# gardnerzhou/CHAP

Hardware: AMD Instinct MI355X
Metric: training volumes/sec (2D 256^2 bs24) (higher is better)
Workload: dtype bf16; 1 GPU; ACDC 2D DualDecoder bs=24 (12 lab + 12 unlab) 256x256, 1 perturb step(s), N_v=U; global_batch=24, parallelism=dp1, hip_graph=True, losses_finite=True

## Files before the change

### chap_amd/csrc/actbwd_math.h

```cpp
#pragma once
#include "common.h"

typedef float actbwd_f32x2 __attribute__((ext_vector_type(2)));

__device__ __forceinline__ void actbwd_consts8(const float a0[8], const float a1[8], const float gm[8], const float mean[8], const float istd[8], float count,
                                               float k0[8], float cB[8], float cC[8]) {
#pragma unroll
    for (int j = 0; j < 8; ++j) {
        k0[j] = gm[j] * istd[j];
        const float k1 = a0[j] / count, k2 = a1[j] / count;
        cB[j] = -istd[j] * k0[j] * k2;
        cC[j] = __builtin_fmaf(mean[j] * istd[j] * k0[j], k2, -k0[j] * k1);
    }
}

__device__ __forceinline__ void actbwd_deriv8(const float raw[8], const float dy[8], const float sa[8], const float sb[8], bool act, float slope, float dz[8]) {
    if (act) {
#pragma unroll
        for (int j = 0; j < 4; ++j) {
            const actbwd_f32x2 r2 = {raw[2 * j], raw[2 * j + 1]}, a2 = {sa[2 * j], sa[2 * j + 1]}, b2 = {sb[2 * j], sb[2 * j + 1]};
            const actbwd_f32x2 z = __builtin_elementwise_fma(r2, a2, b2);
            const actbwd_f32x2 f = {z.x > 0.f ? 1.f : slope, z.y > 0.f ? 1.f : slope};
            const actbwd_f32x2 g2 = {dy[2 * j], dy[2 * j + 1]};
            const actbwd_f32x2 d = g2 * f;
            dz[2 * j] = d.x; dz[2 * j + 1] = d.y;
        }
    } else {
#pragma unroll
        for (int j = 0; j < 8; ++j) dz[j] = dy[j];
    }
}
__device__ __forceinline__ void actbwd_keep8(float dz[8], uint2 m, float keep_scale) {
#pragma unroll
    for (int j = 0; j < 8; ++j) {
        const uint32_t w = j < 4 ? m.x : m.y;
        dz[j] = ((w >> (8 * (j & 3))) & 0xff) ? dz[j] * keep_scale : 0.f;
    }
}

__device__ __forceinline__ void actbwd_apply8(const float dz[8], const float raw[8], const float k0[8], const float cB[8], const float cC[8], float o[8]) {
#pragma unroll
    for (int j = 0; j < 4; ++j) {
        const actbwd_f32x2 d = {dz[2 * j], dz[2 * j + 1]}, r2 = {raw[2 * j], raw[2 * j + 1]};
        const actbwd_f32x2 A = {k0[2 * j], k0[2 * j + 1]}, B = {cB[2 * j], cB[2 * j + 1]}, Cc = {cC[2 * j], cC[2 * j + 1]};
        const actbwd_f32x2 r = __builtin_elementwise_fma(d, A, __builtin_elementwise_fma(r2, B, Cc));
        o[2 * j] = r.x; o[2 * j + 1] = r.y;
    }
}
```

### chap_amd/csrc/pointwise.hip

```cpp
#include <cstdlib>
#include "common.h"
#include "launch.h"
#include "actbwd_math.h"
#include "conv_c1_mfma.h"

typedef unsigned int u32;

__device__ __forceinline__ double wave_sum_f64(double v) {
#pragma unroll
    for (int o = 32; o > 0; o >>= 1) v += __shfl_xor(v, o, 64);
    return v;
}

template <typename T, bool D3, int CO>
__device__ __forceinline__ void conv_c1_fwd_kernel(const chap_conv_c1_params& P) {
    constexpr int KD = D3 ? 3 : 1, TAPS = KD * 9;
    __shared__ float ws[CO * TAPS + 2 * CO];
    __shared__ float bstat[4][2 * CO];
    for (int i = threadIdx.x; i < CO * TAPS; i += 256) ws[i] = P.w[i];
    for (int i = threadIdx.x; i < CO; i += 256) { ws[CO * TAPS + i] = P.bias ? P.bias[i] : 0.f; ws[CO * TAPS + CO + i] = (P.stats && P.stats_shift) ? P.stats_shift[i] : 0.f; }
    __syncthreads();
    const long npix = (long)P.N * P.D * P.H * P.W;
    float ssum[CO], ssq[CO];
#pragma unroll
    for (int c = 0; c < CO; ++c) { ssum[c] = 0.f; ssq[c] = 0.f; }
    for (long pix = (long)blockIdx.x * 256 + threadIdx.x; pix < npix; pix += (long)gridDim.x * 256) {
        const u32 up = (u32)pix;
        const int x = (int)(up % (u32)P.W); u32 r = up / (u32)P.W;
        const int y = (int)(r % (u32)P.H); r /= (u32)P.H;
        const int z = (int)(r % (u32)P.D); const int n = (int)(r / (u32)P.D);
        float in[TAPS];
#pragma unroll
        for (int dz = 0; dz < KD; ++dz)
#pragma unroll
            for (int dy = 0; dy < 3; ++dy)
#pragma unroll
                for (int dx = 0; dx < 3; ++dx) {
                    const int zz = z + dz - (D3 ? 1 : 0), yy = y + dy - 1, xx = x + dx - 1;
                    const bool ib = (unsigned)zz < (unsigned)P.D && (unsigned)yy < (unsigned)P.H && (unsigned)xx < (unsigned)P.W;
                    in[(dz * 3 + dy) * 3 + dx] = ib ? P.x[(((long)n * P.D + zz) * P.H + yy) * P.W + xx] : 0.f;
                }
        float acc[CO];
#pragma unroll
        for (int c = 0; c < CO; ++c) {
            float a = ws[CO * TAPS + c];
#pragma unroll
            for (int t = 0; t < TAPS; ++t) a = fmaf(in[t], ws[c * TAPS + t], a);
            acc[c] = a;
            const float as = a - ws[CO * TAPS + CO + c];
            ssum[c] += as; ssq[c] += as * as;
        }
        T* o = (T*)P.out + pix * CO;
#pragma unroll
        for (int c = 0; c < CO; c += 8) st8(o + c, acc + c);
    }
    if (P.stats) {
#pragma unroll
        for (int c = 0; c < CO; ++c) {
            const float s = wave_sum(ssum[c]), q = wave_sum(ssq[c]);
            if ((threadIdx.x & 63) == 0) { bstat[threadIdx.x >> 6][c] = s; bstat[threadIdx.x >> 6][CO + c] = q; }
        }
        __syncthreads();
        if (blockIdx.x == 0 && threadIdx.x == 0) *(int*)P.stats = (int)gridDim.x;
        for (int i = threadIdx.x; i < 2 * CO; i += 256)
// ... 112 lines not shown
            P.ws[(long)blockIdx.x * (CO * TAPS + CO) + i] = part[0][i] + part[1][i] + part[2][i] + part[3][i];
    }
}

struct c1_reduce_args { const float* ws; int nblocks, taps; float* dw; float* db; };
template <int CO>
__device__ __forceinline__ void conv_c1_reduce_kernel(const c1_reduce_args& A) {
    const float* ws = A.ws; const int nblocks = A.nblocks, taps = A.taps; float* dw = A.dw; float* db = A.db;
    __shared__ float red[4];
    const int i = blockIdx.x;
    const int tot = CO * taps + CO;
    float s = 0.f;
    for (int b = threadIdx.x; b < nblocks; b += 256) s += ws[(long)b * tot + i];
    s = wave_sum(s);
    if ((threadIdx.x & 63) == 0) red[threadIdx.x >> 6] = s;
    __syncthreads();
    if (threadIdx.x == 0) {
        s = (red[0] + red[1]) + (red[2] + red[3]);
        if (i < CO * taps) { if (dw) dw[i] += s; } else if (db) db[i - CO * taps] += s;
    }
}

static int c1_bwd_blocks(const chap_conv_c1_bwd_params* p) {
    const long npix = (long)p->N * p->D * p->H * p->W;
    long b = (npix + 255) / 256;
    return (int)(b < 1024 ? b : 1024);
}
extern "C" size_t chap_conv_c1_bwd_ws(const chap_conv_c1_bwd_params* p) {
    const int taps = p->dims == 3 ? 27 : 9;
    return (size_t)c1_bwd_blocks(p) * (p->Cout * taps + p->Cout) * sizeof(float);
}
extern "C" int chap_conv_c1_bwd(const chap_conv_c1_bwd_params* p, void* stream) {
    CHAP_CHECK_ARG(p && p->g && p->w, "chap_conv_c1_bwd: null argument");
    CHAP_CHECK_ARG(p->Cout == 16, "chap_conv_c1_bwd: Cout=%d (only 16 built)", p->Cout);
    CHAP_CHECK_ARG(!(p->dw || p->db) || (p->ws && p->x), "chap_conv_c1_bwd: dw/db need x and ws");
    const int nb = c1_bwd_blocks(p);
    hipStream_t s = (hipStream_t)stream;
    const bool d3 = p->dims == 3, bf = p->dtype == CHAP_BF16;
    const c1_bwd_args a = {*p, nb};
    int r;
    if (bf && d3) r = chap_launch<c1_bwd_args, conv_c1_bwd_kernel<bf16_t, true, 16>, 256>(dim3(nb), dim3(256), 0, s, a, "chap_conv_c1_bwd");
    else if (bf) r = chap_launch<c1_bwd_args, conv_c1_bwd_kernel<bf16_t, false, 16>, 256>(dim3(nb), dim3(256), 0, s, a, "chap_conv_c1_bwd");
    else if (d3) r = chap_launch<c1_bwd_args, conv_c1_bwd_kernel<float, true, 16>, 256>(dim3(nb), dim3(256), 0, s, a, "chap_conv_c1_bwd");
    else r = chap_launch<c1_bwd_args, conv_c1_bwd_kernel<float, false, 16>, 256>(dim3(nb), dim3(256), 0, s, a, "chap_conv_c1_bwd");
    if (r) return r;
    if (p->dw || p->db) {
        const int taps = d3 ? 27 : 9, tot = 16 * taps + 16;
        const c1_reduce_args ra = {(const float*)p->ws, nb, taps, p->dw, p->db};
        return chap_launch<c1_reduce_args, conv_c1_reduce_kernel<16>, 256>(dim3(tot), dim3(256), 0, s, ra, "chap_conv_c1_bwd(reduce)");
    }
    return CHAP_OK;
}

__device__ __forceinline__ void bn_finalize_kernel(const chap_bn_finalize_params& P) {
    const int c = blockIdx.x * 4 + (threadIdx.x >> 6), lane = threadIdx.x & 63;
    if (c >= P.C) return;
    const int nslots = *(const int*)P.stats;
    const bool upd = P.momentum > 0.f && P.running_mean;
    const float gam = P.gamma[c], bet = P.beta[c], sft = P.stats_shift ? P.stats_shift[c] : 0.f;
    const float rm0 = upd ? P.running_mean[c] : 0.f, rv0 = upd ? P.running_var[c] : 0.f;
    const int nsub = P.Clog / P.C;
    const float* st = P.stats + CHAP_STATS_HDR;
    double s = 0.0, q = 0.0;
    constexpr int NB = CHAP_STATS_MAX_SLOTS / 64;
    for (int k = 0; k < nsub; ++k) {
        float vs[NB], vq[NB];
#pragma unroll
        for (int i = 0; i < NB; ++i) {
            const int b = lane + 64 * i;
            const float* row = st + (long)(b < nslots ? b : 0) * 2 * P.Clog + k * P.C + c;
            vs[i] = row[0]; vq[i] = row[P.Clog];
        }
#pragma unroll
        for (int i = 0; i < NB; ++i) {
            const bool ok = lane + 64 * i < nslots;
            s += ok ? (double)vs[i] : 0.0; q += ok ? (double)vq[i] : 0.0;
        }
    }
    s = wave_sum_f64(s); q = wave_sum_f64(q);
    if (lane != 0) return;
    if (c == 0 && P.num_batches_tracked && P.momentum > 0.f) *P.num_batches_tracked += 1;
    const double cnt = (double)P.count;
    const double ms = s / cnt;
    double var = q / cnt - ms * ms;
    var = var > 0.0 ? var : 0.0;
    const float mean = (float)((double)sft + ms);
    const float invstd = (float)(1.0 / sqrt(var + (double)P.eps));
    const float sc = gam * invstd;
    P.scale[c] = sc;
    P.shift[c] = bet - mean * sc;
    if (P.mean) { P.mean[c] = mean; P.invstd[c] = invstd; }
    if (upd) {
        const float unb = (float)(cnt > 1.0 ? var * cnt / (cnt - 1.0) : var);
        P.running_mean[c] = (1.f - P.momentum) * rm0 + P.momentum * mean;
        P.running_var[c] = (1.f - P.momentum) * rv0 + P.momentum * unb;
    }
}
extern "C" int chap_bn_finalize(const chap_bn_finalize_params* p, void* stream) {
    CHAP_CHECK_ARG(p && p->stats && p->gamma && p->beta && p->scale && p->shift && p->C > 0 && p->count > 0, "chap_bn_finalize: bad argument");
    CHAP_CHECK_ARG(p->Clog >= p->C && p->Clog % p->C == 0, "chap_bn_finalize: Clog=%d must be a multiple of C=%d", p->Clog, p->C);
    if (chap_lab_skip(KNOB_LAB_SKIP_BNFIN)) return CHAP_OK;
    return chap_launch<chap_bn_finalize_params, bn_finalize_kernel, 256>(dim3(cdiv(p->C, 4)), dim3(256), 0, (hipStream_t)stream, *p, "chap_bn_finalize");
}

__device__ __forceinline__ void bn_eval_kernel(const chap_bn_eval_params& P) {
    const int c = blockIdx.x * blockDim.x + threadIdx.x;
    if (c >= P.C) return;
    const float sc = P.gamma[c] * rsqrtf(P.running_var[c] + P.eps);
    P.scale[c] = sc;
    P.shift[c] = P.beta[c] - P.running_mean[c] * sc;
}
extern "C" int chap_bn_eval_affine(const chap_bn_eval_params* p, void* stream) {
    CHAP_CHECK_ARG(p && p->gamma && p->beta && p->running_mean && p->running_var && p->scale && p->shift && p->C > 0, "chap_bn_eval_affine: bad argument");
    return chap_launch<chap_bn_eval_params, bn_eval_kernel, 64>(dim3(cdiv(p->C, 64)), dim3(64), 0, (hipStream_t)stream, *p, "chap_bn_eval_affine");
}

template <typename T>
__device__ __forceinline__ void act_pool2_kernel(const chap_pool_params& P) {
    const int D = P.D > 1 ? P.D : 1, KZ = P.D > 1 ? 2 : 1;
    const int C8 = P.r.C / 8, OD = D / KZ, OH = P.H / 2, OW = P.W / 2;
    const long total = (long)P.N * OD * OH * OW * C8;
    for (long i = (long)blockIdx.x * 256 + threadIdx.x; i < total; i += (long)gridDim.x * 256) {
        const u32 ui = (u32)i;
        const int c8 = (int)(ui % (u32)C8) * 8; u32 r = ui / (u32)C8;
        const int ox = (int)(r % (u32)OW); r /= (u32)OW;
        const int oy = (int)(r % (u32)OH); r /= (u32)OH;
        const int oz = (int)(r % (u32)OD); const int n = (int)(r / (u32)OD);
        float best[8]; uint32_t bi[8];
        for (int k = 0; k < 4 * KZ; ++k) {
            const long pix = (((long)n * D + KZ * oz + (k >> 2)) * P.H + 2 * oy + ((k >> 1) & 1)) * P.W + 2 * ox + (k & 1);
            float v[8];
            src_load8<T>(P.r, n, pix, c8, v);
#pragma unroll
            for (int j = 0; j < 8; ++j)
                if (k == 0 || v[j] > best[j] || v[j] != v[j]) { best[j] = v[j]; bi[j] = k; }
        }
        const long op = (((long)n * OD + oz) * OH + oy) * OW + ox;
        st8((T*)P.out + op * P.r.C + c8, best);
        if (P.idx) {
            uint2 m;
            m.x = bi[0] | (bi[1] << 8) | (bi[2] << 16) | (bi[3] << 24);
            m.y = bi[4] | (bi[5] << 8) | (bi[6] << 16) | (bi[7] << 24);
            *(uint2*)(P.idx + op * P.r.C + c8) = m;
        }
    }
}
extern "C" int chap_act_pool2(const chap_pool_params* p, void* stream) {
    CHAP_CHECK_ARG(p && p->r.ptr && p->out, "chap_act_pool2: null argument");
// ... 146 lines not shown
    for (long i = (long)blockIdx.x * 256 + threadIdx.x; i < total; i += (long)gridDim.x * 256) {
        const u32 ui = (u32)i;
        const int c8 = (int)(ui % (u32)C8) * 8; u32 r = ui / (u32)C8;
        const int x = (int)(r % (u32)P.W); r /= (u32)P.W;
        const int y = (int)(r % (u32)P.H); r /= (u32)P.H;
        const int z = (int)(r % (u32)P.D); const int n = (int)(r / (u32)P.D);
        float acc[8];
#pragma unroll
        for (int j = 0; j < 8; ++j) acc[j] = 0.f;
        int oz_[5], oy_[5]; float wz_[5], wy_[5];
        int nz = 1; oz_[0] = z; wz_[0] = 1.f;
        if (P.dims == 3) nz = up_axis_adjoint(z, P.D, OD, oz_, wz_);
        const int ny = up_axis_adjoint(y, P.H, OH, oy_, wy_);
        int ox_[5]; float wx_[5];
#pragma unroll
        for (int k = 0; k < 5; ++k) {
            const int o = 2 * x - 2 + k, oc = min(max(o, 0), OW - 1);
            int a0, a1; float w1;
            ac_coord(oc, P.W, OW, a0, a1, w1);
            const float w = (a0 == x ? 1.f - w1 : 0.f) + (a1 == x ? w1 : 0.f);
            ox_[k] = oc; wx_[k] = (o == oc) ? w : 0.f;
        }
        for (int a = 0; a < nz; ++a)
            for (int b = 0; b < ny; ++b) {
                const long row = (((long)n * OD + oz_[a]) * OH + oy_[b]) * OW;
                const float wzy = wz_[a] * wy_[b];
                float v[5][8];
#pragma unroll
                for (int c = 0; c < 5; ++c) ld8(g + (row + ox_[c]) * P.g_ld + P.g_coff + c8, v[c]);
#pragma unroll
                for (int c = 0; c < 5; ++c) {
                    const float w = wzy * wx_[c];
                    if (wx_[c] != 0.f) {
#pragma unroll
                        for (int j = 0; j < 8; ++j) acc[j] = fmaf(w, v[c][j], acc[j]);
                    }
                }
            }
        const long cp = (((long)n * P.D + z) * P.H + y) * P.W + x;
        st8((T*)P.out + cp * P.C + c8, acc);
    }
}
extern "C" int chap_upsample2x_bwd(const chap_upsample_bwd_params* p, void* stream) {
    CHAP_CHECK_ARG(p && p->g && p->out && p->C % 8 == 0 && p->g_ld % 8 == 0 && p->g_coff % 8 == 0, "chap_upsample2x_bwd: bad argument");
    if (chap_lab_skip(KNOB_LAB_SKIP_UPSAMPLE_BWD)) return CHAP_OK;
    const long total = (long)p->N * p->D * p->H * p->W * (p->C / 8);
    const int blocks = chap_blocks(total, 8192);
    if (p->dtype == CHAP_BF16) return chap_launch<chap_upsample_bwd_params, upsample2x_bwd_kernel<bf16_t>, 256>(dim3(blocks), dim3(256), 0, (hipStream_t)stream, *p, "chap_upsample2x_bwd");
    return chap_launch<chap_upsample_bwd_params, upsample2x_bwd_kernel<float>, 256>(dim3(blocks), dim3(256), 0, (hipStream_t)stream, *p, "chap_upsample2x_bwd");
}

typedef float f32x2 __attribute__((ext_vector_type(2)));

template <typename T>
__device__ __forceinline__ void act_bwd_dz(const chap_act_bwd_params& P, const float sa[8], const float sb[8], int n, long pix, int y, int x, int c8,
                                           float raw[8], float dz[8]) {
    const chap_src_t& s = P.r;
    const int C = s.C;
    ld8((const T*)s.ptr + pix * s.ld + s.coff + c8, raw);
    float gsum[8];
#pragma unroll
    for (int j = 0; j < 8; ++j) gsum[j] = 0.f;
    for (int k = 0; k < P.ng; ++k) {
        float v[8];
        ld8((const T*)P.g[k] + pix * P.g_ld[k] + P.g_coff[k] + c8, v);
#pragma unroll
        for (int j = 0; j < 8; ++j) gsum[j] += v[j];
    }
    if (P.g_pool) {
        const int OH = P.H / 2, OW = P.W / 2;
        const long pp = ((long)n * OH + (y >> 1)) * OW + (x >> 1);
        const uint32_t me = ((y & 1) << 1) | (x & 1);
        float v[8];
        ld8((const T*)P.g_pool + pp * C + c8, v);
        const uint2 m = *(const uint2*)(P.pool_idx + pp * C + c8);
#pragma unroll
        for (int j = 0; j < 8; ++j) {
            const uint32_t w = j < 4 ? m.x : m.y;
            if (((w >> (8 * (j & 3))) & 0xff) == me) gsum[j] += v[j];
        }
    }
    actbwd_deriv8(raw, gsum, sa, sb, s.act != 0, s.slope, dz);
    if (s.keep) actbwd_keep8(dz, *(const uint2*)(s.keep + pix * C + c8), s.keep_scale);
    if (s.chan_mul) {
        float cm[8];
        ld8(s.chan_mul + (long)n * C + c8, cm);
#pragma unroll
        for (int j = 0; j < 8; ++j) dz[j] *= cm[j];
    }
}

template <typename T, bool APPLY>
__device__ __forceinline__ void act_bwd_kernel(const chap_act_bwd_params& P) {
    extern __shared__ float red[];
    const int C = P.r.C, C8 = C / 8;
    const long npix = (long)P.N * P.D * P.H * P.W;
    const int c8 = (threadIdx.x % C8) * 8;
    const int prow = threadIdx.x / C8, PPB = 256 / C8;
    float s0[8], s1[8], mean[8], istd[8], k0[8], sa[8], sb[8], cB[8], cC[8], cM[8];
#pragma unroll
    for (int j = 0; j < 8; ++j) { s0[j] = 0.f; s1[j] = 0.f; sa[j] = 1.f; sb[j] = 0.f; }
    if (P.r.scale) { ld8(P.r.scale + c8, sa); ld8(P.r.shift + c8, sb); }
#pragma unroll
    for (int j = 0; j < 8; ++j) { k0[j] = 1.f; mean[j] = 0.f; istd[j] = 1.f; }
    if (P.bn) { ld8(P.mean + c8, mean); ld8(P.invstd + c8, istd); }
#pragma unroll
    for (int j = 0; j < 8; ++j) { cB[j] = 0.f; cC[j] = 0.f; cM[j] = -mean[j] * istd[j]; }
    if (APPLY) {
        if (P.bn == 1) {
            for (int i = threadIdx.x; i < 2 * C; i += 256) red[i] = P.sums[i];
            __syncthreads();
            float gm[8], a0[8], a1[8];
            ld8(P.gamma + c8, gm);
#pragma unroll
            for (int j = 0; j < 8; ++j) { a0[j] = red[c8 + j]; a1[j] = red[C + c8 + j]; }
            actbwd_consts8(a0, a1, gm, mean, istd, P.count, k0, cB, cC);
        } else if (P.r.scale) {
            ld8(P.r.scale + c8, k0);
        }
    }
    const bool need_coords = P.g_pool != nullptr || P.r.chan_mul != nullptr;
    if (prow < PPB) {
        for (long pix = (long)blockIdx.x * PPB + prow; pix < npix; pix += (long)gridDim.x * PPB) {
            int x = 0, y = 0, n = 0;
            if (need_coords) {
                const u32 up = (u32)pix;
                x = (int)(up % (u32)P.W); u32 r = up / (u32)P.W;
                y = (int)(r % (u32)P.H); r /= (u32)P.H;
                n = (int)(r / (u32)P.D);
            }
            float raw[8], dz[8];
            act_bwd_dz<T>(P, sa, sb, n, pix, y, x, c8, raw, dz);
            if (!APPLY) {
#pragma unroll
                for (int j = 0; j < 4; ++j) {
                    const f32x2 d = {dz[2 * j], dz[2 * j + 1]}, r2 = {raw[2 * j], raw[2 * j + 1]};
                    const f32x2 i2 = {istd[2 * j], istd[2 * j + 1]}, m2 = {cM[2 * j], cM[2 * j + 1]};
                    const f32x2 xh = r2 * i2 + m2;
                    f32x2 a = {s0[2 * j], s0[2 * j + 1]}, b = {s1[2 * j], s1[2 * j + 1]};
                    a = a + d; b = d * xh + b;
                    s0[2 * j] = a.x; s0[2 * j + 1] = a.y; s1[2 * j] = b.x; s1[2 * j + 1] = b.y;
                }
            } else {
                float o[8];
                actbwd_apply8(dz, raw, k0, cB, cC, o);
                st8((T*)P.gout + pix * C + c8, o);
            }
        }
    }
    if (!APPLY) {
        for (int i = threadIdx.x; i < 4 * 2 * C; i += 256) red[i] = 0.f;
        __syncthreads();
        const int wave = threadIdx.x >> 6;
#pragma unroll
        for (int j = 0; j < 8; ++j) {
            float a = s0[j], b = s1[j];
            if (C8 == 1) { a = row16_sum(a); b = row16_sum(b); }
            else if (C8 == 2) { a = row16_stride_sum<2>(a); b = row16_stride_sum<2>(b); }
            else if (C8 == 4) { a = row16_stride_sum<4>(a); b = row16_stride_sum<4>(b); }
            else if (C8 == 8) { a = row16_stride_sum<8>(a); b = row16_stride_sum<8>(b); }
            for (int o = (C8 > 16 ? C8 : 16); o < 64; o <<= 1) { a += __shfl_xor(a, o, 64); b += __shfl_xor(b, o, 64); }
            if ((threadIdx.x & 63) < C8 && prow < PPB) { red[(wave * 2 + 0) * C + c8 + j] = a; red[(wave * 2 + 1) * C + c8 + j] = b; }
        }
        __syncthreads();
        float* dst = P.sums + (long)(1 + blockIdx.x) * 2 * C;
        for (int i = threadIdx.x; i < 2 * C; i += 256) {
            const int which = i / C, c = i % C;
            dst[i] = (red[(0 * 2 + which) * C + c] + red[(1 * 2 + which) * C + c]) + (red[(2 * 2 + which) * C + c] + red[(3 * 2 + which) * C + c]);
        }
    }
}

struct act_bwd_sum_args { float* sums; int nblocks; float* dgamma; float* dbeta; int C; };
__device__ __forceinline__ void act_bwd_sum_kernel(const act_bwd_sum_args& A) {
    float* sums = A.sums; const int nblocks = A.nblocks; float* dgamma = A.dgamma; float* dbeta = A.dbeta; const int C = A.C;
    const int i = blockIdx.x * 4 + (threadIdx.x >> 6), lane = threadIdx.x & 63;
    if (i >= 2 * C) return;
    double t = 0.0;
    constexpr int NB = CHAP_ACT_BWD_SLOTS / 64;
    float vv[NB];
#pragma unroll
    for (int k = 0; k < NB; ++k) {
        const int b = lane + 64 * k;
        vv[k] = sums[(long)(1 + (b < nblocks ? b : 0)) * 2 * C + i];
    }
#pragma unroll
    for (int k = 0; k < NB; ++k) t += (lane + 64 * k < nblocks) ? (double)vv[k] : 0.0;
    t = wave_sum_f64(t);
    if (lane != 0) return;
    const float v = (float)t;
    sums[i] = v;
    if (i < C) { if (dbeta) dbeta[i] += v; } else if (dgamma) dgamma[i - C] += v;
}

static int act_bwd_check(const chap_act_bwd_params* p) {
    CHAP_CHECK_ARG(p && p->r.ptr, "chap_act_bwd: null argument");
    CHAP_CHECK_ARG(p->r.C % 8 == 0 && 256 % (p->r.C / 8) == 0 && p->r.C <= 1024, "chap_act_bwd: C=%d unsupported", p->r.C);
    CHAP_CHECK_ARG(p->ng >= 0 && p->ng <= 3, "chap_act_bwd: ng=%d", p->ng);
    CHAP_CHECK_ARG(p->bn >= 0 && p->bn <= 2, "chap_act_bwd: bn=%d", p->bn);
    CHAP_CHECK_ARG(p->bn != 1 || (p->mean && p->invstd && p->gamma && p->sums), "chap_act_bwd: bn=1 needs mean/invstd/gamma/sums");
    CHAP_CHECK_ARG(!p->g_pool || (p->pool_idx && p->D == 1 && p->H % 2 == 0 && p->W % 2 == 0), "chap_act_bwd: pooled gradient needs idx and even 2D dims");
    return CHAP_OK;
}
static int act_bwd_blocks(const chap_act_bwd_params* p) {
    const long npix = (long)p->N * p->D * p->H * p->W;
    const int ppb = 256 / (p->r.C / 8);
    long b = (npix + ppb - 1) / ppb;
    long cap = chap_knob(KNOB_ACTBWD_BLOCKS);
    if (cap > CHAP_ACT_BWD_SLOTS) cap = 512;
    return (int)(b < cap ? b : cap);
}
extern "C" int chap_act_bwd_reduce(const chap_act_bwd_params* p, void* stream) {
    int r = act_bwd_check(p); if (r) return r;
    CHAP_CHECK_ARG(p->bn && p->mean && p->invstd && p->sums, "chap_act_bwd_reduce: needs bn, mean, invstd, sums");
    const size_t lds = 4 * 2 * p->r.C * sizeof(float);
    const int nb = act_bwd_blocks(p);
    if (p->dtype == CHAP_BF16) r = chap_launch<chap_act_bwd_params, act_bwd_kernel<bf16_t, false>, 256>(dim3(nb), dim3(256), lds, (hipStream_t)stream, *p, "chap_act_bwd_reduce");
    else r = chap_launch<chap_act_bwd_params, act_bwd_kernel<float, false>, 256>(dim3(nb), dim3(256), lds, (hipStream_t)stream, *p, "chap_act_bwd_reduce");
    if (r) return r;
    if (chap_lab_skip(KNOB_LAB_SKIP_ACTSUM)) return CHAP_OK;
    const act_bwd_sum_args sa = {p->sums, nb, p->dgamma, p->dbeta, p->r.C};
    return chap_launch<act_bwd_sum_args, act_bwd_sum_kernel, 256>(dim3(cdiv(2 * p->r.C, 4)), dim3(256), 0, (hipStream_t)stream, sa, "chap_act_bwd_reduce(sum)");
}
extern "C" int chap_act_bwd_apply(const chap_act_bwd_params* p, void* stream) {
    int r = act_bwd_check(p); if (r) return r;
    CHAP_CHECK_ARG(p->gout, "chap_act_bwd_apply: null gout");
    if (chap_lab_skip(KNOB_LAB_SKIP_ACTAPPLY) && p->bn == 1) return CHAP_OK;
    const size_t lds = 2 * p->r.C * sizeof(float);
    if (p->dtype == CHAP_BF16) return chap_launch<chap_act_bwd_params, act_bwd_kernel<bf16_t, true>, 256>(dim3(act_bwd_blocks(p)), dim3(256), lds, (hipStream_t)stream, *p, "chap_act_bwd_apply");
    return chap_launch<chap_act_bwd_params, act_bwd_kernel<float, true>, 256>(dim3(act_bwd_blocks(p)), dim3(256), lds, (hipStream_t)stream, *p, "chap_act_bwd_apply");
}

template <typename T>
__device__ __forceinline__ void planar_to_cl_kernel(const chap_planar_to_cl_params& P) {
    const int Cp = P.Cpad > P.C ? P.Cpad : P.C;
    const long total = (long)P.N * P.P * Cp;
    for (long i = (long)blockIdx.x * blockDim.x + threadIdx.x; i < total; i += (long)gridDim.x * blockDim.x) {
        const u32 ui = (u32)i;
        const int c = (int)(ui % (u32)Cp); const u32 r = ui / (u32)Cp;
        const long pp = r % (u32)P.P; const int n = (int)(r / (u32)P.P);
        const float v = c < P.C ? P.in[((long)n * P.C + c) * P.P + pp] : 0.f;
        ((T*)P.out)[(n * (long)P.P + pp) * P.out_ld + P.out_coff + c] = elem<T>::put(v);
    }
}
template <typename T>
__device__ __forceinline__ void planar_to_cl8_kernel(const chap_planar_to_cl_params& P) {
    const int Cp = P.Cpad > P.C ? P.Cpad : P.C, C8 = Cp / 8;
    const long total = (long)P.N * P.P * C8;
    for (long i = (long)blockIdx.x * 256 + threadIdx.x; i < total; i += (long)gridDim.x * 256) {
        const u32 ui = (u32)i;
        const int c8 = (int)(ui % (u32)C8) * 8; const u32 r = ui / (u32)C8;
        const long pp = r % (u32)P.P; const int n = (int)(r / (u32)P.P);
        float v[8];
#pragma unroll
        for (int j = 0; j < 8; ++j) v[j] = c8 + j < P.C ? P.in[((long)n * P.C + c8 + j) * P.P + pp] : 0.f;
        st8((T*)P.out + (n * (long)P.P + pp) * P.out_ld + P.out_coff + c8, v);
    }
}
extern "C" int chap_planar_to_cl(const chap_planar_to_cl_params* p, void* stream) {
    CHAP_CHECK_ARG(p && p->in && p->out, "chap_planar_to_cl: null argument");
    const int Cp = p->Cpad > p->C ? p->Cpad : p->C;
    if (Cp % 8 == 0 && p->out_ld % 8 == 0 && p->out_coff % 8 == 0) {
        const long total = (long)p->N * p->P * (Cp / 8);
        const int blocks = chap_blocks(total, 16384);
        if (p->dtype == CHAP_BF16) return chap_launch<chap_planar_to_cl_params, planar_to_cl8_kernel<bf16_t>, 256>(dim3(blocks), dim3(256), 0, (hipStream_t)stream, *p, "chap_planar_to_cl");
        return chap_launch<chap_planar_to_cl_params, planar_to_cl8_kernel<float>, 256>(dim3(blocks), dim3(256), 0, (hipStream_t)stream, *p, "chap_planar_to_cl");
    }
    const long total = (long)p->N * p->P * Cp;
    const int blocks = chap_blocks(total, 4096);
    if (p->dtype == CHAP_BF16) return chap_launch<chap_planar_to_cl_params, planar_to_cl_kernel<bf16_t>, 256>(dim3(blocks), dim3(256), 0, (hipStream_t)stream, *p, "chap_planar_to_cl");
    return chap_launch<chap_planar_to_cl_params, planar_to_cl_kernel<float>, 256>(dim3(blocks), dim3(256), 0, (hipStream_t)stream, *p, "chap_planar_to_cl");
}

template <typename T>
__device__ __forceinline__ void cl_to_planar_kernel(const chap_cl_to_planar_params& P) {
    const int C = P.r.C;
    const long total = (long)P.N * P.P * C;
    for (long i = (long)blockIdx.x * blockDim.x + threadIdx.x; i < total; i += (long)gridDim.x * blockDim.x) {
        const u32 ui = (u32)i;
        const long pp = ui % (u32)P.P; const u32 r = ui / (u32)P.P;
        const int c = (int)(r % (u32)C); const int n = (int)(r / (u32)C);
        P.out[i] = src_load1<T>(P.r, n, (long)n * P.P + pp, c);
    }
// ... 59 lines not shown
```

Baseline: 4070 volumes/s.

## Restructure activation-backward kernels with software-pipelined loads and specialized fast path

Rewrites the activation/BN backward reduce and apply kernels so each thread precomputes a per-source address plan and prefetches the next pixel's inputs (raw, grads, keep mask, pool, channel multiplier) while computing the current one. Adds a non-generic template specialization for the common single-gradient, no-pool, no-chan-mul case. Uses explicit global address-space pointers, keeps kernel arguments in scalar registers, and drops the LDS staging of sums in the apply path, which no longer needs dynamic shared memory. Also adds a check that tensors stay under 4 GB so 32-bit offsets can be used. This adds register pressure from the double-buffered loads.

```diff
diff --git a/chap_amd/csrc/actbwd_math.h b/chap_amd/csrc/actbwd_math.h
--- a/chap_amd/csrc/actbwd_math.h
+++ b/chap_amd/csrc/actbwd_math.h
@@ -3,15 +3,16 @@
 
 typedef float actbwd_f32x2 __attribute__((ext_vector_type(2)));
 
+__device__ __forceinline__ void actbwd_consts1(float a0, float a1, float gm, float mean, float istd, float count, float& k0, float& cB, float& cC) {
+    k0 = gm * istd;
+    const float k1 = a0 / count, k2 = a1 / count;
+    cB = -istd * k0 * k2;
+    cC = __builtin_fmaf(mean * istd * k0, k2, -k0 * k1);
+}
 __device__ __forceinline__ void actbwd_consts8(const float a0[8], const float a1[8], const float gm[8], const float mean[8], const float istd[8], float count,
                                                float k0[8], float cB[8], float cC[8]) {
 #pragma unroll
-    for (int j = 0; j < 8; ++j) {
-        k0[j] = gm[j] * istd[j];
-        const float k1 = a0[j] / count, k2 = a1[j] / count;
-        cB[j] = -istd[j] * k0[j] * k2;
-        cC[j] = __builtin_fmaf(mean[j] * istd[j] * k0[j], k2, -k0[j] * k1);
-    }
+    for (int j = 0; j < 8; ++j) actbwd_consts1(a0[j], a1[j], gm[j], mean[j], istd[j], count, k0[j], cB[j], cC[j]);
 }
 
 __device__ __forceinline__ void actbwd_deriv8(const float raw[8], const float dy[8], const float sa[8], const float sb[8], bool act, float slope, float dz[8]) {
diff --git a/chap_amd/csrc/pointwise.hip b/chap_amd/csrc/pointwise.hip
--- a/chap_amd/csrc/pointwise.hip
+++ b/chap_amd/csrc/pointwise.hip
@@ -10,6 +10,34 @@
 #pragma unroll
     for (int o = 32; o > 0; o >>= 1) v += __shfl_xor(v, o, 64);
     return v;
+}
+
+template <typename A>
+__device__ __forceinline__ A chap_args_once(const A& p) {
+    static_assert(sizeof(A) % 4 == 0, "argument block is not a whole number of words");
+    struct words { uint32_t w[sizeof(A) / 4]; };
+    words w = __builtin_bit_cast(words, p);
+#pragma unroll
+    for (unsigned i = 0; i < sizeof(A) / 4; ++i) asm volatile("" : "+s"(w.w[i]));
+    return __builtin_bit_cast(A, w);
+}
+#define CHAP_GLOBAL __attribute__((address_space(1)))
+typedef const CHAP_GLOBAL char* chap_gptr;
+typedef float f32x4n __attribute__((ext_vector_type(4)));
+typedef uint32_t u32x4n __attribute__((ext_vector_type(4)));
+typedef uint32_t u32x2n __attribute__((ext_vector_type(2)));
+template <typename X> __device__ __forceinline__ chap_gptr chap_global(const X* p) { return (chap_gptr)p; }
+template <typename V> __device__ __forceinline__ V ldg(chap_gptr p) { return *(const CHAP_GLOBAL V*)p; }
+__device__ __forceinline__ void ld8g(chap_gptr p, float v[8]) {
+    const f32x4n a = ldg<f32x4n>(p), b = ldg<f32x4n>(p + 16);
+    v[0] = a.x; v[1] = a.y; v[2] = a.z; v[3] = a.w; v[4] = b.x; v[5] = b.y; v[6] = b.z; v[7] = b.w;
+}
+__device__ __forceinline__ void st8g(CHAP_GLOBAL float* p, const float v[8]) {
+    *(CHAP_GLOBAL f32x4n*)p = f32x4n{v[0], v[1], v[2], v[3]};
+    *(CHAP_GLOBAL f32x4n*)(p + 4) = f32x4n{v[4], v[5], v[6], v[7]};
+}
+__device__ __forceinline__ void st8g(CHAP_GLOBAL bf16_t* p, const float v[8]) {
+    *(CHAP_GLOBAL u32x4n*)p = u32x4n{pack2bf(v[0], v[1]), pack2bf(v[2], v[3]), pack2bf(v[4], v[5]), pack2bf(v[6], v[7])};
 }
 
 template <typename T, bool D3, int CO>
@@ -228,15 +256,17 @@
     return CHAP_OK;
 }
 
-__device__ __forceinline__ void bn_finalize_kernel(const chap_bn_finalize_params& P) {
+__device__ __forceinline__ void bn_finalize_kernel(const chap_bn_finalize_params& Pk) {
+    const chap_bn_finalize_params P = chap_args_once(Pk);
+    typedef const CHAP_GLOBAL float* gf;
     const int c = blockIdx.x * 4 + (threadIdx.x >> 6), lane = threadIdx.x & 63;
     if (c >= P.C) return;
-    const int nslots = *(const int*)P.stats;
+    const int nslots = *(const CHAP_GLOBAL int*)P.stats;
     const bool upd = P.momentum > 0.f && P.running_mean;
-    const float gam = P.gamma[c], bet = P.beta[c], sft = P.stats_shift ? P.stats_shift[c] : 0.f;
-    const float rm0 = upd ? P.running_mean[c] : 0.f, rv0 = upd ? P.running_var[c] : 0.f;
+    const float gam = ((gf)P.gamma)[c], bet = ((gf)P.beta)[c], sft = P.stats_shift ? ((gf)P.stats_shift)[c] : 0.f;
+    const float rm0 = upd ? ((gf)P.running_mean)[c] : 0.f, rv0 = upd ? ((gf)P.running_var)[c] : 0.f;
     const int nsub = P.Clog / P.C;
-    const float* st = P.stats + CHAP_STATS_HDR;
+    const gf st = (gf)P.stats + CHAP_STATS_HDR;
     double s = 0.0, q = 0.0;
     constexpr int NB = CHAP_STATS_MAX_SLOTS / 64;
     for (int k = 0; k < nsub; ++k) {
@@ -244,7 +274,7 @@
 #pragma unroll
         for (int i = 0; i < NB; ++i) {
             const int b = lane + 64 * i;
-            const float* row = st + (long)(b < nslots ? b : 0) * 2 * P.Clog + k * P.C + c;
+            const gf row = st + (long)(b < nslots ? b : 0) * 2 * P.Clog + k * P.C + c;
             vs[i] = row[0]; vq[i] = row[P.Clog];
         }
 #pragma unroll
@@ -255,7 +285,7 @@
     }
     s = wave_sum_f64(s); q = wave_sum_f64(q);
     if (lane != 0) return;
-    if (c == 0 && P.num_batches_tracked && P.momentum > 0.f) *P.num_batches_tracked += 1;
+    if (c == 0 && P.num_batches_tracked && P.momentum > 0.f) *(CHAP_GLOBAL int64_t*)P.num_batches_tracked += 1;
     const double cnt = (double)P.count;
     const double ms = s / cnt;
     double var = q / cnt - ms * ms;
@@ -263,13 +293,14 @@
     const float mean = (float)((double)sft + ms);
     const float invstd = (float)(1.0 / sqrt(var + (double)P.eps));
     const float sc = gam * invstd;
-    P.scale[c] = sc;
-    P.shift[c] = bet - mean * sc;
-    if (P.mean) { P.mean[c] = mean; P.invstd[c] = invstd; }
+    typedef CHAP_GLOBAL float* gw;
+    ((gw)P.scale)[c] = sc;
+    ((gw)P.shift)[c] = bet - mean * sc;
+    if (P.mean) { ((gw)P.mean)[c] = mean; ((gw)P.invstd)[c] = invstd; }
     if (upd) {
         const float unb = (float)(cnt > 1.0 ? var * cnt / (cnt - 1.0) : var);
-        P.running_mean[c] = (1.f - P.momentum) * rm0 + P.momentum * mean;
-        P.running_var[c] = (1.f - P.momentum) * rv0 + P.momentum * unb;
+        ((gw)P.running_mean)[c] = (1.f - P.momentum) * rm0 + P.momentum * mean;
+        ((gw)P.running_var)[c] = (1.f - P.momentum) * rv0 + P.momentum * unb;
     }
 }
 extern "C" int chap_bn_finalize(const chap_bn_finalize_params* p, void* stream) {
@@ -522,101 +553,198 @@
 
 typedef float f32x2 __attribute__((ext_vector_type(2)));
 
+template <typename T> struct act_pk;
+template <> struct act_pk<bf16_t> { u32x4n v; };
+template <> struct act_pk<float> { f32x4n a, b; };
+__device__ __forceinline__ void pk_ld(chap_gptr p, act_pk<bf16_t>& r) { r.v = ldg<u32x4n>(p); }
+__device__ __forceinline__ void pk_ld(chap_gptr p, act_pk<float>& r) { r.a = ldg<f32x4n>(p); r.b = ldg<f32x4n>(p + 16); }
+__device__ __forceinline__ void pk_unpack(const act_pk<bf16_t>& r, float v[8]) {
+    v[0] = __uint_as_float(r.v.x << 16); v[1] = __uint_as_float(r.v.x & 0xffff0000u);
+    v[2] = __uint_as_float(r.v.y << 16); v[3] = __uint_as_float(r.v.y & 0xffff0000u);
+    v[4] = __uint_as_float(r.v.z << 16); v[5] = __uint_as_float(r.v.z & 0xffff0000u);
+    v[6] = __uint_as_float(r.v.w << 16); v[7] = __uint_as_float(r.v.w & 0xffff0000u);
+}
+__device__ __forceinline__ void pk_unpack(const act_pk<float>& r, float v[8]) {
+    v[0] = r.a.x; v[1] = r.a.y; v[2] = r.a.z; v[3] = r.a.w; v[4] = r.b.x; v[5] = r.b.y; v[6] = r.b.z; v[7] = r.b.w;
+}
+
+struct act_src1 { chap_gptr base; u32 stride; };
+struct act_plan {
+    act_src1 raw, g[3], gp, idx, keep, cm;
+    bool has_g[3], has_pool, has_keep, has_cm, need_coords, act;
+    int cm_hi;
+    int W, H, D;
+    float slope, keep_scale;
+};
 template <typename T>
-__device__ __forceinline__ void act_bwd_dz(const chap_act_bwd_params& P, const float sa[8], const float sb[8], int n, long pix, int y, int x, int c8,
-                                           float raw[8], float dz[8]) {
-    const chap_src_t& s = P.r;
-    const int C = s.C;
-    ld8((const T*)s.ptr + pix * s.ld + s.coff + c8, raw);
-    float gsum[8];
+__device__ __forceinline__ act_plan act_make_plan(const chap_act_bwd_params& P) {
+    constexpr u32 ES = sizeof(T);
+    act_plan S;
+    const u32 C = (u32)P.r.C;
+    S.raw = {chap_global(P.r.ptr) + (long)P.r.coff * ES, (u32)P.r.ld * ES};
+#pragma unroll
+    for (int k = 0; k < 3; ++k) {
+        S.has_g[k] = k < P.ng;
+        S.g[k] = S.has_g[k] ? act_src1{chap_global(P.g[k]) + (long)P.g_coff[k] * ES, (u32)P.g_ld[k] * ES} : S.raw;
+    }
+    S.has_pool = P.g_pool != nullptr; S.has_keep = P.r.keep != nullptr; S.has_cm = P.r.chan_mul != nullptr;
+    S.gp = S.has_pool ? act_src1{chap_global(P.g_pool), C * ES} : S.raw;
+    S.idx = S.has_pool ? act_src1{chap_global(P.pool_idx), C} : S.raw;
+    S.keep = S.has_keep ? act_src1{chap_global(P.r.keep), C} : S.raw;
+    S.cm = S.has_cm ? act_src1{chap_global(P.r.chan_mul), C * 4} : S.raw;
+    S.cm_hi = S.has_cm ? 16 : 0;
+    S.need_coords = S.has_pool || S.has_cm;
+    S.act = P.r.act != 0;
+    S.W = P.W; S.H = P.H; S.D = P.D;
+    S.slope = P.r.slope; S.keep_scale = P.r.keep_scale;
+    return S;
+}
+struct act_lane { int t, b, cm; };
+
+template <typename T> struct act_trip { act_pk<T> raw, g0, g1, g2, gp; u32x2n idx, keep; f32x4n cm0, cm1; uint32_t me; };
+
+__device__ __forceinline__ chap_gptr act_addr(const act_src1& s, u32 i, int lane) { return s.base + (u32)(i * s.stride + (u32)lane); }
+template <typename T, bool GEN>
+__device__ __forceinline__ void act_issue(const act_plan& S, const act_lane& L, u32 pix, act_trip<T>& t) {
+    if (GEN) {
+        u32 pidx = pix, nidx = pix;
+        t.me = 0;
+        if (S.need_coords) {
+            const u32 up = pix;
+            const int x = (int)(up % (u32)S.W); u32 r = up / (u32)S.W;
+            const int y = (int)(r % (u32)S.H); r /= (u32)S.H;
+            const int n = (int)(r / (u32)S.D);
+            const int OH = S.H / 2, OW = S.W / 2;
+            const u32 pp = ((u32)n * OH + (y >> 1)) * OW + (x >> 1);
+            t.me = ((y & 1) << 1) | (x & 1);
+            pidx = S.has_pool ? pp : pix; nidx = S.has_cm ? (u32)n : pix;
+        }
+        pk_ld(act_addr(S.g[0], pix, L.t), t.g0);
+        pk_ld(act_addr(S.g[1], pix, L.t), t.g1);
+        pk_ld(act_addr(S.g[2], pix, L.t), t.g2);
+        pk_ld(act_addr(S.gp, pidx, L.t), t.gp);
+        t.idx = ldg<u32x2n>(act_addr(S.idx, pidx, L.b));
+        const chap_gptr cp = act_addr(S.cm, nidx, L.cm);
+        t.cm0 = ldg<f32x4n>(cp); t.cm1 = ldg<f32x4n>(cp + S.cm_hi);
+    } else {
+        pk_ld(act_addr(S.g[0], pix, L.t), t.g0);
+    }
+    t.keep = ldg<u32x2n>(act_addr(S.keep, pix, L.b));
+    pk_ld(act_addr(S.raw, pix, L.t), t.raw);
+}
+
+template <typename T, bool GEN>
+__device__ __forceinline__ void act_gsum(const act_plan& S, const act_trip<T>& t, float gsum[8]) {
+    float v[8];
 #pragma unroll
     for (int j = 0; j < 8; ++j) gsum[j] = 0.f;
-    for (int k = 0; k < P.ng; ++k) {
-        float v[8];
-        ld8((const T*)P.g[k] + pix * P.g_ld[k] + P.g_coff[k] + c8, v);
+    if (!GEN || S.has_g[0]) {
+        pk_unpack(t.g0, v);
 #pragma unroll
         for (int j = 0; j < 8; ++j) gsum[j] += v[j];
     }
-    if (P.g_pool) {
-        const int OH = P.H / 2, OW = P.W / 2;
-        const long pp = ((long)n * OH + (y >> 1)) * OW + (x >> 1);
-        const uint32_t me = ((y & 1) << 1) | (x & 1);
-        float v[8];
-        ld8((const T*)P.g_pool + pp * C + c8, v);
-        const uint2 m = *(const uint2*)(P.pool_idx + pp * C + c8);
+    if (GEN) {
+        if (S.has_g[1]) {
+            pk_unpack(t.g1, v);
+#pragma unroll
+            for (int j = 0; j < 8; ++j) gsum[j] += v[j];
+        }
+        if (S.has_g[2]) {
+            pk_unpack(t.g2, v);
+#pragma unroll
+            for (int j = 0; j < 8; ++j) gsum[j] += v[j];
+        }
+        if (S.has_pool) {
+            pk_unpack(t.gp, v);
+#pragma unroll
+            for (int j = 0; j < 8; ++j) {
+                const uint32_t w = j < 4 ? t.idx.x : t.idx.y;
+                if (((w >> (8 * (j & 3))) & 0xff) == t.me) gsum[j] += v[j];
+            }
+        }
+    }
+}
+template <typename T, bool GEN>
+__device__ __forceinline__ void act_bwd_dz(const act_plan& S, const act_trip<T>& t, const float gsum[8], const float sa[8], const float sb[8], float raw[8], float dz[8]) {
+    pk_unpack(t.raw, raw);
+    actbwd_deriv8(raw, gsum, sa, sb, S.act, S.slope, dz);
+    if (S.has_keep) actbwd_keep8(dz, make_uint2(t.keep.x, t.keep.y), S.keep_scale);
+    if (GEN && S.has_cm) {
+        const float cm[8] = {t.cm0.x, t.cm0.y, t.cm0.z, t.cm0.w, t.cm1.x, t.cm1.y, t.cm1.z, t.cm1.w};
+#pragma unroll
+        for (int j = 0; j < 8; ++j) dz[j] *= cm[j];
+    }
+}
+
+template <typename T, bool APPLY, bool GEN>
+__device__ __forceinline__ void act_bwd_kernel(const chap_act_bwd_params& Pk) {
+    extern __shared__ float red[];
+    const chap_act_bwd_params P = chap_args_once(Pk);
+    const act_plan S = act_make_plan<T>(P);
+    const int C = P.r.C, C8 = C / 8, bn = P.bn;
+    const long npix = (long)P.N * P.D * P.H * P.W;
+    const chap_gptr scale = chap_global(P.r.scale), shift = chap_global(P.r.shift);
+    const chap_gptr meanp = chap_global(P.mean), istdp = chap_global(P.invstd), gammap = chap_global(P.gamma);
+    CHAP_GLOBAL float* const sums = (CHAP_GLOBAL float*)P.sums; CHAP_GLOBAL T* const gout = (CHAP_GLOBAL T*)P.gout;
+    const float count = P.count;
+    const int c8 = (threadIdx.x % C8) * 8;
+    float s0[8], s1[8], istd[8], k0[8], sa[8], sb[8], cB[8], cC[8], cM[8];
+#pragma unroll
+    for (int j = 0; j < 8; ++j) { s0[j] = 0.f; s1[j] = 0.f; sa[j] = 1.f; sb[j] = 0.f; k0[j] = 1.f; istd[j] = 1.f; cB[j] = 0.f; cC[j] = 0.f; cM[j] = 0.f; }
+    if (APPLY && bn == 1) {
+        float mean[8], gm[8], a0[8], a1[8];
+        ld8g(meanp + c8 * 4, mean); ld8g(istdp + c8 * 4, istd); ld8g(gammap + c8 * 4, gm);
+        ld8g((chap_gptr)(sums + c8), a0); ld8g((chap_gptr)(sums + C + c8), a1);
 #pragma unroll
         for (int j = 0; j < 8; ++j) {
-            const uint32_t w = j < 4 ? m.x : m.y;
-            if (((w >> (8 * (j & 3))) & 0xff) == me) gsum[j] += v[j];
-        }
-    }
-    actbwd_deriv8(raw, gsum, sa, sb, s.act != 0, s.slope, dz);
-    if (s.keep) actbwd_keep8(dz, *(const uint2*)(s.keep + pix * C + c8), s.keep_scale);
-    if (s.chan_mul) {
-        float cm[8];
-        ld8(s.chan_mul + (long)n * C + c8, cm);
-#pragma unroll
-        for (int j = 0; j < 8; ++j) dz[j] *= cm[j];
-    }
-}
-
-template <typename T, bool APPLY>
-__device__ __forceinline__ void act_bwd_kernel(const chap_act_bwd_params& P) {
-    extern __shared__ float red[];
-    const int C = P.r.C, C8 = C / 8;
-    const long npix = (long)P.N * P.D * P.H * P.W;
-    const int c8 = (threadIdx.x % C8) * 8;
+            actbwd_consts1(a0[j], a1[j], gm[j], mean[j], istd[j], count, k0[j], cB[j], cC[j]);
+            __builtin_amdgcn_sched_barrier(0);
+        }
+    }
     const int prow = threadIdx.x / C8, PPB = 256 / C8;
-    float s0[8], s1[8], mean[8], istd[8], k0[8], sa[8], sb[8], cB[8], cC[8], cM[8];
-#pragma unroll
-    for (int j = 0; j < 8; ++j) { s0[j] = 0.f; s1[j] = 0.f; sa[j] = 1.f; sb[j] = 0.f; }
-    if (P.r.scale) { ld8(P.r.scale + c8, sa); ld8(P.r.shift + c8, sb); }
-#pragma unroll
-    for (int j = 0; j < 8; ++j) { k0[j] = 1.f; mean[j] = 0.f; istd[j] = 1.f; }
-    if (P.bn) { ld8(P.mean + c8, mean); ld8(P.invstd + c8, istd); }
-#pragma unroll
-    for (int j = 0; j < 8; ++j) { cB[j] = 0.f; cC[j] = 0.f; cM[j] = -mean[j] * istd[j]; }
-    if (APPLY) {
-        if (P.bn == 1) {
-            for (int i = threadIdx.x; i < 2 * C; i += 256) red[i] = P.sums[i];
-            __syncthreads();
-            float gm[8], a0[8], a1[8];
-            ld8(P.gamma + c8, gm);
-#pragma unroll
-            for (int j = 0; j < 8; ++j) { a0[j] = red[c8 + j]; a1[j] = red[C + c8 + j]; }
-            actbwd_consts8(a0, a1, gm, mean, istd, P.count, k0, cB, cC);
-        } else if (P.r.scale) {
-            ld8(P.r.scale + c8, k0);
-        }
-    }
-    const bool need_coords = P.g_pool != nullptr || P.r.chan_mul != nullptr;
-    if (prow < PPB) {
-        for (long pix = (long)blockIdx.x * PPB + prow; pix < npix; pix += (long)gridDim.x * PPB) {
-            int x = 0, y = 0, n = 0;
-            if (need_coords) {
-                const u32 up = (u32)pix;
-                x = (int)(up % (u32)P.W); u32 r = up / (u32)P.W;
-                y = (int)(r % (u32)P.H); r /= (u32)P.H;
-                n = (int)(r / (u32)P.D);
+    const act_lane L = {c8 * (int)sizeof(T), c8, S.has_cm ? c8 * 4 : c8 * (int)sizeof(T)};
+    long pix = (long)blockIdx.x * PPB + prow;
+    const long step = (long)gridDim.x * PPB, last = npix - 1;
+    if (scale) { ld8g(scale + c8 * 4, sa); ld8g(shift + c8 * 4, sb); }
+    constexpr bool CM_FIRST = GEN && sizeof(T) == 4;
+    float mean[8];
+    if (!APPLY) { ld8g(meanp + c8 * 4, mean); ld8g(istdp + c8 * 4, istd); }
+    if (!APPLY && CM_FIRST) {
+#pragma unroll
+        for (int j = 0; j < 8; ++j) cM[j] = -mean[j] * istd[j];
+    }
+    act_trip<T> cur;
+    act_issue<T, GEN>(S, L, (u32)(pix < last ? pix : last), cur);
+    if (!APPLY && !CM_FIRST) {
+        __builtin_amdgcn_sched_barrier(0);
+#pragma unroll
+        for (int j = 0; j < 8; ++j) cM[j] = -mean[j] * istd[j];
+    }
+    if (APPLY && bn != 1 && scale) {
+#pragma unroll
+        for (int j = 0; j < 8; ++j) k0[j] = sa[j];
+    }
+    for (; pix < npix; pix += step) {
+        float raw[8], dz[8], gsum[8];
+        act_gsum<T, GEN>(S, cur, gsum);
+        act_bwd_dz<T, GEN>(S, cur, gsum, sa, sb, raw, dz);
+        if (!APPLY) {
+#pragma unroll
+            for (int j = 0; j < 4; ++j) {
+                const f32x2 d = {dz[2 * j], dz[2 * j + 1]}, r2 = {raw[2 * j], raw[2 * j + 1]};
+                const f32x2 i2 = {istd[2 * j], istd[2 * j + 1]}, m2 = {cM[2 * j], cM[2 * j + 1]};
+                const f32x2 xh = r2 * i2 + m2;
+                f32x2 a = {s0[2 * j], s0[2 * j + 1]}, b = {s1[2 * j], s1[2 * j + 1]};
+                a = a + d; b = d * xh + b;
+                s0[2 * j] = a.x; s0[2 * j + 1] = a.y; s1[2 * j] = b.x; s1[2 * j + 1] = b.y;
             }
-            float raw[8], dz[8];
-            act_bwd_dz<T>(P, sa, sb, n, pix, y, x, c8, raw, dz);
-            if (!APPLY) {
-#pragma unroll
-                for (int j = 0; j < 4; ++j) {
-                    const f32x2 d = {dz[2 * j], dz[2 * j + 1]}, r2 = {raw[2 * j], raw[2 * j + 1]};
-                    const f32x2 i2 = {istd[2 * j], istd[2 * j + 1]}, m2 = {cM[2 * j], cM[2 * j + 1]};
-                    const f32x2 xh = r2 * i2 + m2;
-                    f32x2 a = {s0[2 * j], s0[2 * j + 1]}, b = {s1[2 * j], s1[2 * j + 1]};
-                    a = a + d; b = d * xh + b;
-                    s0[2 * j] = a.x; s0[2 * j + 1] = a.y; s1[2 * j] = b.x; s1[2 * j + 1] = b.y;
-                }
-            } else {
-                float o[8];
-                actbwd_apply8(dz, raw, k0, cB, cC, o);
-                st8((T*)P.gout + pix * C + c8, o);
-            }
-        }
+        } else {
+            float o[8];
+            actbwd_apply8(dz, raw, k0, cB, cC, o);
+            st8g(gout + pix * C + c8, o);
+        }
+        const long pn = pix + step < last ? pix + step : last;
+        act_issue<T, GEN>(S, L, (u32)pn, cur);
     }
     if (!APPLY) {
         for (int i = threadIdx.x; i < 4 * 2 * C; i += 256) red[i] = 0.f;
@@ -630,10 +758,10 @@
             else if (C8 == 4) { a = row16_stride_sum<4>(a); b = row16_stride_sum<4>(b); }
             else if (C8 == 8) { a = row16_stride_sum<8>(a); b = row16_stride_sum<8>(b); }
             for (int o = (C8 > 16 ? C8 : 16); o < 64; o <<= 1) { a += __shfl_xor(a, o, 64); b += __shfl_xor(b, o, 64); }
-            if ((threadIdx.x & 63) < C8 && prow < PPB) { red[(wave * 2 + 0) * C + c8 + j] = a; red[(wave * 2 + 1) * C + c8 + j] = b; }
+            if ((threadIdx.x & 63) < C8) { red[(wave * 2 + 0) * C + c8 + j] = a; red[(wave * 2 + 1) * C + c8 + j] = b; }
         }
         __syncthreads();
-        float* dst = P.sums + (long)(1 + blockIdx.x) * 2 * C;
+        CHAP_GLOBAL float* dst = sums + (long)(1 + blockIdx.x) * 2 * C;
         for (int i = threadIdx.x; i < 2 * C; i += 256) {
             const int which = i / C, c = i % C;
             dst[i] = (red[(0 * 2 + which) * C + c] + red[(1 * 2 + which) * C + c]) + (red[(2 * 2 + which) * C + c] + red[(3 * 2 + which) * C + c]);
@@ -642,10 +770,15 @@
 }
 
 struct act_bwd_sum_args { float* sums; int nblocks; float* dgamma; float* dbeta; int C; };
-__device__ __forceinline__ void act_bwd_sum_kernel(const act_bwd_sum_args& A) {
-    float* sums = A.sums; const int nblocks = A.nblocks; float* dgamma = A.dgamma; float* dbeta = A.dbeta; const int C = A.C;
+__device__ __forceinline__ void act_bwd_sum_kernel(const act_bwd_sum_args& Ak) {
+    const act_bwd_sum_args A = chap_args_once(Ak);
+    CHAP_GLOBAL float* const sums = (CHAP_GLOBAL float*)A.sums; const int nblocks = A.nblocks, C = A.C;
     const int i = blockIdx.x * 4 + (threadIdx.x >> 6), lane = threadIdx.x & 63;
     if (i >= 2 * C) return;
+    CHAP_GLOBAL float* const acc = (CHAP_GLOBAL float*)(i < C ? A.dbeta : A.dgamma);
+    const int ai = i < C ? i : i - C;
+    float prior = 0.f;
+    if (acc) prior = acc[ai];
     double t = 0.0;
     constexpr int NB = CHAP_ACT_BWD_SLOTS / 64;
     float vv[NB];
@@ -660,13 +793,19 @@
     if (lane != 0) return;
     const float v = (float)t;
     sums[i] = v;
-    if (i < C) { if (dbeta) dbeta[i] += v; } else if (dgamma) dgamma[i - C] += v;
+    if (acc) acc[ai] = prior + v;
 }
 
 static int act_bwd_check(const chap_act_bwd_params* p) {
     CHAP_CHECK_ARG(p && p->r.ptr, "chap_act_bwd: null argument");
     CHAP_CHECK_ARG(p->r.C % 8 == 0 && 256 % (p->r.C / 8) == 0 && p->r.C <= 1024, "chap_act_bwd: C=%d unsupported", p->r.C);
     CHAP_CHECK_ARG(p->ng >= 0 && p->ng <= 3, "chap_act_bwd: ng=%d", p->ng);
+    {
+        long ld = p->r.ld > p->r.C ? p->r.ld : p->r.C;
+        for (int k = 0; k < p->ng; ++k) ld = p->g_ld[k] > ld ? p->g_ld[k] : ld;
+        const long bytes = (long)p->N * p->D * p->H * p->W * ld * (p->dtype == CHAP_BF16 ? 2 : 4);
+        CHAP_CHECK_ARG(bytes < (1l << 32), "chap_act_bwd: a tensor of %ld bytes (4 GB at most)", bytes);
+    }
     CHAP_CHECK_ARG(p->bn >= 0 && p->bn <= 2, "chap_act_bwd: bn=%d", p->bn);
     CHAP_CHECK_ARG(p->bn != 1 || (p->mean && p->invstd && p->gamma && p->sums), "chap_act_bwd: bn=1 needs mean/invstd/gamma/sums");
     CHAP_CHECK_ARG(!p->g_pool || (p->pool_idx && p->D == 1 && p->H % 2 == 0 && p->W % 2 == 0), "chap_act_bwd: pooled gradient needs idx and even 2D dims");
@@ -680,13 +819,21 @@
     if (cap > CHAP_ACT_BWD_SLOTS) cap = 512;
     return (int)(b < cap ? b : cap);
 }
+template <typename T, bool APPLY>
+static int act_bwd_launch_t(const chap_act_bwd_params* p, int nb, size_t lds, hipStream_t s, const char* name) {
+    if (p->ng == 1 && !p->g_pool && !p->r.chan_mul) return chap_launch<chap_act_bwd_params, act_bwd_kernel<T, APPLY, false>, 256>(dim3(nb), dim3(256), lds, s, *p, name);
+    return chap_launch<chap_act_bwd_params, act_bwd_kernel<T, APPLY, true>, 256>(dim3(nb), dim3(256), lds, s, *p, name);
+}
+template <bool APPLY>
+static int act_bwd_launch(const chap_act_bwd_params* p, int nb, size_t lds, hipStream_t s, const char* name) {
+    return p->dtype == CHAP_BF16 ? act_bwd_launch_t<bf16_t, APPLY>(p, nb, lds, s, name) : act_bwd_launch_t<float, APPLY>(p, nb, lds, s, name);
+}
 extern "C" int chap_act_bwd_reduce(const chap_act_bwd_params* p, void* stream) {
     int r = act_bwd_check(p); if (r) return r;
     CHAP_CHECK_ARG(p->bn && p->mean && p->invstd && p->sums, "chap_act_bwd_reduce: needs bn, mean, invstd, sums");
     const size_t lds = 4 * 2 * p->r.C * sizeof(float);
     const int nb = act_bwd_blocks(p);
-    if (p->dtype == CHAP_BF16) r = chap_launch<chap_act_bwd_params, act_bwd_kernel<bf16_t, false>, 256>(dim3(nb), dim3(256), lds, (hipStream_t)stream, *p, "chap_act_bwd_reduce");
-    else r = chap_launch<chap_act_bwd_params, act_bwd_kernel<float, false>, 256>(dim3(nb), dim3(256), lds, (hipStream_t)stream, *p, "chap_act_bwd_reduce");
+    r = act_bwd_launch<false>(p, nb, lds, (hipStream_t)stream, "chap_act_bwd_reduce");
     if (r) return r;
     if (chap_lab_skip(KNOB_LAB_SKIP_ACTSUM)) return CHAP_OK;
     const act_bwd_sum_args sa = {p->sums, nb, p->dgamma, p->dbeta, p->r.C};
@@ -696,9 +843,7 @@
     int r = act_bwd_check(p); if (r) return r;
     CHAP_CHECK_ARG(p->gout, "chap_act_bwd_apply: null gout");
     if (chap_lab_skip(KNOB_LAB_SKIP_ACTAPPLY) && p->bn == 1) return CHAP_OK;
-    const size_t lds = 2 * p->r.C * sizeof(float);
-    if (p->dtype == CHAP_BF16) return chap_launch<chap_act_bwd_params, act_bwd_kernel<bf16_t, true>, 256>(dim3(act_bwd_blocks(p)), dim3(256), lds, (hipStream_t)stream, *p, "chap_act_bwd_apply");
-    return chap_launch<chap_act_bwd_params, act_bwd_kernel<float, true>, 256>(dim3(act_bwd_blocks(p)), dim3(256), lds, (hipStream_t)stream, *p, "chap_act_bwd_apply");
+    return act_bwd_launch<true>(p, act_bwd_blocks(p), 0, (hipStream_t)stream, "chap_act_bwd_apply");
 }
 
 template <typename T>
```

Result: faster. 4157 volumes/s (median of 6 runs) (+2.1%).
